# RuanJohn/Mava

Measured on AMD Instinct MI355X. Metric: env-steps/sec (whole node), ff_mappo RWARE tiny-4ag, higher is better.
Workload: dtype f32 via 2 x f16 split operands on the MFMA (3 products, f32 accumulate); 1 GPU; ff_mappo RWARE tiny-4ag-shaped synthetic obs, 4096 envs/GPU (update_batch_size=1 x num_envs=4096), rollout_length=128, ppo_epochs=4, num_minibatches=2, agents=4, obs=70/264, actions=5, one step = one PPO update = 524288 env-steps per GPU; parallelism=dp1

## Files before the change

### include/mava_hip.h

```cpp
#ifndef MAVA_HIP_H
#define MAVA_HIP_H

#include <stddef.h>
#include <stdint.h>

#ifdef __cplusplus
extern "C" {
#endif

typedef struct ihipStream_t* mava_stream_t;

const char* mava_last_error(void);
int mava_abi_version(void);

typedef struct mava_ctx mava_ctx;
enum {
  MAVA_CTX_MATMUL_MODE = 0,
  MAVA_CTX_CRITIC_AGGREGATION = 1,
  MAVA_CTX_GAE_VARIANT = 2,
  MAVA_CTX_POLICY_VARIANT = 3,
  MAVA_CTX_H2_LAUNCHES = 4,
  MAVA_CTX_TRAIN_VARIANT = 5,
  MAVA_CTX_W8_LAUNCHES = 6,
  MAVA_CTX_W1_SPLIT_FRESH = 7,
  MAVA_CTX_EXACT_TILES = 8,
  MAVA_CTX_X16_LAUNCHES = 9,
  MAVA_CTX_X16_W8_LAUNCHES = 10
};
int mava_ctx_create(mava_ctx** out);
int mava_ctx_destroy(mava_ctx* ctx);
int mava_ctx_set(mava_ctx* ctx, int key, long value);
int mava_ctx_get(const mava_ctx* ctx, int key, long* value);

int mava_gae_f32(const mava_ctx* ctx, const float* reward, const float* value, const uint8_t* done,
                 const float* last_val, const uint8_t* last_done, int T, int N, float gamma,
                 float lambda, float* adv, float* tgt, mava_stream_t s);

int mava_permutation_i32(long n, uint64_t seed, uint64_t counter, int32_t* out, mava_stream_t s);
int mava_permutation_batched_i32(long n, uint64_t seed, uint64_t counter, int n_perm, int32_t* out, long out_stride,
                                 mava_stream_t s);

int mava_clip_adam(float* p, const float* g, float* m, float* v, int32_t* count,
                   const int* seg_off, const float* seg_lr, int n_seg, float grad_scale,
                   float max_norm, int decay, int steps_per_update, int num_updates, float b1,
                   float b2, float eps, const float* loss_sums, float vf_coef, float ent_coef,
                   float* metrics_out, mava_stream_t s);

size_t mava_ppo_finish_workspace_bytes(int Pa, int Pc);
int mava_ppo_finish_f32(mava_ctx* ctx, const float* slab_a, long stride_a, const float* slab_c, long stride_c, int n_slab,
                        int Pa, int Pc, float* g, float* p, float* m, float* v, int32_t* count, float lr_a, float lr_c,
// ... 400 lines not shown
```

### mava_amd/_lib.py

```python
from __future__ import annotations

import ctypes as C
import os
from typing import Optional

import torch

_HERE = os.path.dirname(os.path.abspath(__file__))
LIB_PATH = os.environ.get("MAVA_LIB_PATH") or os.path.join(_HERE, "libmavahip.so")

_lib: Optional[C.CDLL] = None


class MavaHipError(RuntimeError):
    pass


vp = C.c_void_p
i32 = C.c_int
u32 = C.c_uint32
u64 = C.c_uint64
f32 = C.c_float
lng = C.c_long

# ... 116 lines not shown
    global _lib
    if _lib is None:
        if not os.path.exists(LIB_PATH):
            raise MavaHipError(
                f"{LIB_PATH} is missing: build it with `python -m mava_amd.build` "
                "(hipcc --offload-arch=gfx950). There is no CPU fallback."
            )
        _lib = C.CDLL(LIB_PATH)
        _lib.mava_last_error.restype = C.c_char_p
        _lib.mava_last_error.argtypes = []
        for name, args in _SIGNATURES.items():
            fn = getattr(_lib, name)
            fn.argtypes = args
            fn.restype = _RESTYPES.get(name, C.c_int)
    return _lib


class Ctx:

    MATMUL_MODE, CRITIC_AGGREGATION, GAE_VARIANT, POLICY_VARIANT, H2_LAUNCHES, TRAIN_VARIANT, W8_LAUNCHES, W1_SPLIT_FRESH = 0, 1, 2, 3, 4, 5, 6, 7
    EXACT_TILES = 8
    X16_LAUNCHES = 9
    X16_W8_LAUNCHES = 10

    def __init__(self, matmul_mode: str = "f32", critic_aggregation: bool = True):
        if matmul_mode not in ("f32", "f16x2"):
            raise ValueError(f"matmul_mode must be 'f16x2' or 'f32', got {matmul_mode!r}")
        h = C.c_void_p()
        check(lib().mava_ctx_create(C.byref(h)), "mava_ctx_create")
        self.handle: Optional[int] = h.value
        self.set(self.MATMUL_MODE, 1 if matmul_mode == "f16x2" else 0)
        self.set(self.CRITIC_AGGREGATION, int(bool(critic_aggregation)))

    def set(self, key: int, value: int) -> None:
        check(lib().mava_ctx_set(self.handle, key, int(value)), "mava_ctx_set")

    def get(self, key: int) -> int:
        out = C.c_long()
        check(lib().mava_ctx_get(self.handle, key, C.byref(out)), "mava_ctx_get")
        return int(out.value)

    @property
    def matmul_mode(self) -> str:
        return "f16x2" if self.get(self.MATMUL_MODE) == 1 else "f32"

    @property
# ... 51 lines not shown
```

### mava_amd/csrc/api.cpp

```cpp
#include <stdarg.h>
#include <stdio.h>
#include <string.h>

#include "common.h"
#include "ctx.h"

static thread_local char g_err[512] = "";

void mava_set_error(const char* fmt, ...) {
  va_list ap;
  va_start(ap, fmt);
  vsnprintf(g_err, sizeof(g_err), fmt, ap);
  va_end(ap);
}

extern "C" const char* mava_last_error(void) { return g_err; }

extern "C" int mava_abi_version(void) { return 3; }

enum { CTX_MATMUL_MODE = 0, CTX_CRITIC_AGGREGATION = 1, CTX_GAE_VARIANT = 2, CTX_POLICY_VARIANT = 3, CTX_H2_LAUNCHES = 4, CTX_TRAIN_VARIANT = 5, CTX_W8_LAUNCHES = 6, CTX_W1_SPLIT_FRESH = 7, CTX_EXACT_TILES = 8, CTX_X16_LAUNCHES = 9, CTX_X16_W8_LAUNCHES = 10 };

extern "C" int mava_ctx_create(mava_ctx** out) {
  MAVA_ARG_CHECK(out != nullptr, 0, "mava_ctx_create: null output pointer");
  mava_ctx* c = new mava_ctx();
  c->matmul_mode = 0;
  c->critic_aggregation = 1;
  c->gae_variant = 0;
  c->policy_variant = 0;
  c->h2_launches = 0;
  c->train_variant = 0;
  c->w8_launches = 0;
  c->w1_split[0] = c->w1_split[1] = nullptr;
  for (int i = 0; i < 2; ++i) {
    c->w1_fresh[i] = 0;
    c->w1_key_params[i] = nullptr;
    c->w1_key_din[i] = c->w1_key_steps[i] = 0;
  }
  c->exact_tiles = nullptr;
  *out = c;
  return MAVA_OK;
}

extern "C" int mava_ctx_destroy(mava_ctx* c) {
// ... 12 lines not shown
      MAVA_ARG_CHECK(value == 0 || value == 1, 1, "mava_ctx_set: matmul mode %ld (0 = exact f32, 1 = f16x2)", value);
      c->matmul_mode = (int)value;
      c->w1_fresh[0] = c->w1_fresh[1] = 0;
      return MAVA_OK;
    case CTX_CRITIC_AGGREGATION: c->critic_aggregation = value ? 1 : 0; return MAVA_OK;
    case CTX_GAE_VARIANT: c->gae_variant = (int)value; return MAVA_OK;
    case CTX_POLICY_VARIANT: c->policy_variant = (int)value; return MAVA_OK;
    case CTX_H2_LAUNCHES: c->h2_launches = value; return MAVA_OK;
    case CTX_TRAIN_VARIANT: c->train_variant = (int)value; return MAVA_OK;
    case CTX_W8_LAUNCHES: c->w8_launches = value; return MAVA_OK;
    case CTX_W1_SPLIT_FRESH:
      MAVA_ARG_CHECK(value == 0, 1, "mava_ctx_set: MAVA_CTX_W1_SPLIT_FRESH can only be cleared (0) by the caller");
      c->w1_fresh[0] = c->w1_fresh[1] = 0;
      return MAVA_OK;
    case CTX_EXACT_TILES:
      MAVA_ARG_CHECK(value == 0, 1, "mava_ctx_set: MAVA_CTX_EXACT_TILES can only be reset (0) by the caller");
      if (c->exact_tiles != nullptr) {
        MAVA_HIP_CHECK(hipDeviceSynchronize());
        MAVA_HIP_CHECK(hipMemset(c->exact_tiles, 0, sizeof(unsigned long long)));
      }
      return MAVA_OK;
    case CTX_X16_LAUNCHES:
    case CTX_X16_W8_LAUNCHES:
      MAVA_ARG_CHECK(value == 0, 1, "mava_ctx_set: MAVA_CTX_X16_LAUNCHES / _W8_LAUNCHES can only be reset (0) by the caller");
      if (c->exact_tiles != nullptr) {
        MAVA_HIP_CHECK(hipDeviceSynchronize());
        MAVA_HIP_CHECK(hipMemset(c->exact_tiles + (key == CTX_X16_W8_LAUNCHES ? 2 : 1), 0, sizeof(unsigned long long)));
      }
      return MAVA_OK;
    default: mava_set_error("mava_ctx_set: unknown key %d", key); return MAVA_EARG(2);
  }
}

extern "C" int mava_ctx_get(const mava_ctx* c, int key, long* value) {
  MAVA_ARG_CHECK(c != nullptr && value != nullptr, 0, "mava_ctx_get: null argument");
  switch (key) {
    case CTX_MATMUL_MODE: *value = c->matmul_mode; return MAVA_OK;
    case CTX_CRITIC_AGGREGATION: *value = c->critic_aggregation; return MAVA_OK;
    case CTX_GAE_VARIANT: *value = c->gae_variant; return MAVA_OK;
    case CTX_POLICY_VARIANT: *value = c->policy_variant; return MAVA_OK;
    case CTX_H2_LAUNCHES: *value = c->h2_launches; return MAVA_OK;
    case CTX_TRAIN_VARIANT: *value = c->train_variant; return MAVA_OK;
    case CTX_W8_LAUNCHES: *value = c->w8_launches; return MAVA_OK;
    case CTX_W1_SPLIT_FRESH: *value = c->w1_fresh[1]; return MAVA_OK;
    case CTX_EXACT_TILES:
    case CTX_X16_LAUNCHES:
    case CTX_X16_W8_LAUNCHES: {
      unsigned long long n = 0;
      if (c->exact_tiles != nullptr) {
        MAVA_HIP_CHECK(hipDeviceSynchronize());
        MAVA_HIP_CHECK(hipMemcpy(&n, c->exact_tiles + (key == CTX_X16_W8_LAUNCHES ? 2 : key == CTX_X16_LAUNCHES ? 1 : 0), sizeof(n), hipMemcpyDeviceToHost));
      }
      *value = (long)n;
      return MAVA_OK;
    }
    default: mava_set_error("mava_ctx_get: unknown key %d", key); return MAVA_EARG(2);
  }
}
```

### mava_amd/csrc/ppo_train_h2.hip

```cpp
#include "h2_core.h"
#include "ppo_train_task.h"
#include "ctx.h"

#include <type_traits>

#ifndef MAVA_GW_DEPTH
#define MAVA_GW_DEPTH 0
#endif
#define GW_DEPTH MAVA_GW_DEPTH
#ifndef MAVA_GW_DEPTH_WIDE
#define MAVA_GW_DEPTH_WIDE 0
#endif
#ifndef MAVA_P1_EARLY_HALVES
#define MAVA_P1_EARLY_HALVES 2
#endif
#ifndef MAVA_P1_EARLY_RING
#define MAVA_P1_EARLY_RING 3
#endif

namespace {

using namespace h2;

constexpr int STATS_BLOCKS = 128;
// ... 1055 lines not shown
      if (tk.x16_valid != nullptr) x16 = __builtin_amdgcn_readfirstlane((int)*tk.x16_valid) == 1;
    }
    if (X16_CAPABLE && x16) {
      if constexpr (X16_CAPABLE) {
        if (threadIdx.x < 256) {
          h2_body<NO, S1, ACTOR, WIDE, XV, 1, true>(tk, L, w1p, lds);
        } else {
          h2_body<NO, S1, ACTOR, WIDE, XV, 2, true>(tk, L, w1p, lds);
        }
      }
    } else if (threadIdx.x < 256) {
      h2_body<NO, S1, ACTOR, WIDE, XV, 1>(tk, L, w1p, lds);
    } else {
      h2_body<NO, S1, ACTOR, WIDE, XV, 2>(tk, L, w1p, lds);
    }
  } else {
    h2_body<NO, S1, ACTOR, WIDE, XV, 0>(tk, L, w1p, lds);
  }
}

int ctx_counters(mava_ctx* ctx, hipStream_t s) {
  if (ctx->exact_tiles == nullptr) {
    void* word = nullptr;
    MAVA_HIP_CHECK(hipMalloc(&word, 3 * sizeof(unsigned long long)));
    ctx->exact_tiles = static_cast<unsigned long long*>(word);
    MAVA_HIP_CHECK(hipMemsetAsync(word, 0, 3 * sizeof(unsigned long long), s));
  }
  return MAVA_OK;
}

template <int NO, int S1, bool ACTOR, bool WIDE, int XV>
int launch_h2(mava_ctx* ctx, const TrainTask& tk, int n_slab, hipStream_t s) {
  const H2Layout L = make_h2_layout<NO, S1, WIDE>(ACTOR);
  MAVA_ARG_CHECK(L.end <= 163840, 8, "ppo_train_h2: %d bytes of LDS exceed the 160 KiB of a CU", L.end);
  static bool attr_set = false;
  if (!attr_set) {
    MAVA_HIP_CHECK(hipFuncSetAttribute((const void*)ppo_train_h2_kernel<NO, S1, ACTOR, WIDE, XV>,
                                       hipFuncAttributeMaxDynamicSharedMemorySize, L.end));
    attr_set = true;
  }
  const uint4* w1p = nullptr;
  if (WIDE) {
    void*& slot = ctx->w1_split[ACTOR ? 0 : 1];
    if (slot == nullptr) MAVA_HIP_CHECK(hipMalloc(&slot, W1_SPLIT_BYTES));
    uint4* const buf = static_cast<uint4*>(slot);
    const int kind = ACTOR ? 0 : 1;
    int& fresh = ctx->w1_fresh[kind];
    const bool keyed = ctx->w1_key_params[kind] == tk.params && ctx->w1_key_din[kind] == tk.din && ctx->w1_key_steps[kind] == S1;
    if (!(fresh && keyed)) {
// ... 46 lines not shown
    default: return 1;
  }
}

}

static int h2_dispatch(mava_ctx* ctx, const TrainTask& tk, int n_slab, bool actor, hipStream_t s) {
  if (actor) {
    if (tk.action_f != nullptr) return 1;
    if (tk.no <= 8) return dispatch_s1<8, true>(ctx, tk, n_slab, s);
#ifndef MAVA_FAST_BUILD
    if (tk.no <= 16) return dispatch_s1<16, true>(ctx, tk, n_slab, s);
    return dispatch_s1<32, true>(ctx, tk, n_slab, s);
#else
    return 1;
#endif
  }
  return dispatch_s1<1, false>(ctx, tk, n_slab, s);
}

int mava_train_h2_launch(mava_ctx* ctx, const TrainTask& tk_in, int n_slab, bool actor, hipStream_t s) {
  TrainTask tk = tk_in;
  tk.force_xlo = (ctx->train_variant & 2) != 0;
  if ((ctx->train_variant & 1) == 0) {
    if (tk.x16 != nullptr && tk.x16_valid != nullptr) {
      const int rcc = ctx_counters(ctx, s);
      if (rcc != MAVA_OK) return rcc;
      tk.x16_launches = ctx->exact_tiles + 2;
    }
    const int rc8 = mava_train_w8_launch(tk, n_slab, actor, s);
    if (rc8 <= 0) {
      if (rc8 == 0) { ++ctx->h2_launches; ++ctx->w8_launches; }
      return rc8;
    }
  }
  const int rc = h2_dispatch(ctx, tk, n_slab, actor, s);
  if (rc == 0) ++ctx->h2_launches;
  return rc;
}
```

### mava_amd/csrc/ppo_train_task.h

```cpp
#pragma once
#include <stdint.h>

#include "common.h"

struct TrainTask {
  const float* params;
  const float* x;
  int din, no, xshare, xv;
  int A;
  int agg;
  const int32_t* idx;
  long idx_base;
  int Rb;
  const uint8_t* mask;
  const int32_t* action;
  const float* action_f;
  uint32_t seed_lo, seed_hi, ent_step, row_offset;
  float min_scale;
  const float* old_logp;
  const float* adv;
  const double* stats;
  const float* old_value;
  const float* targets;
  float clip_eps, ent_coef, vf_coef;
  float* slab;
  long slab_stride;
  unsigned long long* stamps;
  int force_xlo;
  unsigned long long* exact_tiles;
  const _Float16* x16;
  const uint32_t* x16_valid;
  unsigned long long* x16_launches;
  int x16_ld;
};

struct mava_ctx;
int mava_train_w8_launch(const TrainTask& tk, int n_slab, bool actor, hipStream_t s);
int mava_train_h2_launch(mava_ctx* ctx, const TrainTask& tk, int n_slab, bool actor, hipStream_t s);

extern int g_train_last_instance;
constexpr int train_instance_id(int family, bool actor, bool cont, bool wide, int no, int k, int xv) {
  return family * 1000000 + ((actor ? 1 : 0) + (cont ? 2 : 0) + (wide ? 4 : 0)) * 100000 + no * 1000 + k * 10 + xv;
}
```

### mava_amd/csrc/ppo_train_w8.hip

```cpp
#include "h2_core.h"
#include "ppo_train_task.h"
#include "ctx.h"

namespace {

using namespace h2;
typedef float f32x4 __attribute__((ext_vector_type(4)));

constexpr int STATS_BLOCKS = 128;
#ifndef MAVA_W8_GWD
#define MAVA_W8_GWD 1
#endif
constexpr int GWD = MAVA_W8_GWD;

#ifdef MAVA_STAMPS
#define WSTAMP_DECL unsigned long long ws_prev = __builtin_readcyclecounter(), ws_acc[16] = {0, 0, 0, 0, 0, 0, 0, 0, 0, 0, 0, 0, 0, 0, 0, 0};
#define WSTAMP(i)                                                   \
  do {                                                              \
    __builtin_amdgcn_sched_barrier(0);                              \
    const unsigned long long ws_now = __builtin_readcyclecounter(); \
    ws_acc[i] += ws_now - ws_prev;                                  \
    ws_prev = ws_now;                                               \
    __builtin_amdgcn_sched_barrier(0);                              \
  } while (0)
#else
#define WSTAMP_DECL
#define WSTAMP(i)
#endif

struct Frag4 {
  half4 hi, lo;
};
__device__ __forceinline__ f32x4 mfma3w(const Frag& a, const Frag& b, f32x4 c) {
  c = __builtin_amdgcn_mfma_f32_16x16x32_f16(a.lo, b.hi, c, 0, 0, 0);
  c = __builtin_amdgcn_mfma_f32_16x16x32_f16(a.hi, b.lo, c, 0, 0, 0);
  return __builtin_amdgcn_mfma_f32_16x16x32_f16(a.hi, b.hi, c, 0, 0, 0);
// ... 13 lines not shown
}
__device__ __forceinline__ Frag4 split4(const f32x4& v) {
  Frag4 f;
#pragma unroll
  for (int r = 0; r < 4; ++r) {
    _Float16 a, b;
    split1(v[r], a, b);
    f.hi[r] = a;
    f.lo[r] = b;
  }
  return f;
}

constexpr int WROW = 256;
constexpr int WPLANE32 = 32 * WROW;
constexpr int WIMG = 2 * WPLANE32;
constexpr int W2PLANE = 128 * WROW;
constexpr int DYROW = 48;
constexpr int DYPLANE = 32 * DYROW;
__host__ __device__ inline int w8_sw(int row) { return ((row & 3) << 1) | (((row >> 3) & 1) * 9); }
__host__ __device__ inline int w8_off(int row, int chunk) { return WROW * row + 16 * (chunk ^ w8_sw(row)); }

struct W8Layout {
  int h1, dz2, dz1, w2, xs, dy, small, end;
};
inline W8Layout make_w8_layout() {
  W8Layout L;
  L.h1 = 0;
  L.dz2 = L.h1 + WIMG;
  L.dz1 = L.dz2 + WIMG;
  L.w2 = L.dz1 + WIMG;
  L.xs = L.w2 + 2 * W2PLANE;
  L.dy = L.xs + 2 * WIMG;
  L.small = L.dy + 2 * DYPLANE;
  L.end = L.small + (32 + 16 + 16) * 4;
  return L;
}

template <int NO, int S1, int XV, int W2R, bool ACTOR, int ROLE, bool X16 = false>
__device__ __forceinline__ void w8_body(const TrainTask& tk, const W8Layout& L, u8* lds) {
  constexpr bool DO_LOSS = ROLE != 2, DO_STAGE = ROLE != 1;
  static_assert(!X16 || (DO_STAGE && XV == 2), "the f16 record is read by a staging role of an XV = 2 instance");
  constexpr float WS = ACTOR ? 1.0f : W_SCALE_CRITIC, WU = 1.0f / WS;
  constexpr int KT1 = 2 * S1;
  u8* const H1I = lds + L.h1;
  u8* const DZ2I = lds + L.dz2;
  u8* const DZ1I = lds + L.dz1;
  u8* const W2I = lds + L.w2;
  u8* const DYI = lds + L.dy;
  float* const YP = reinterpret_cast<float*>(lds + L.dz2);
  constexpr int YSTR = (NO == 8) ? 9 : NO;
  float* const B3s = reinterpret_cast<float*>(lds + L.small);
  float* const misc = B3s + 32;
  unsigned* const xflag = reinterpret_cast<unsigned*>(misc + 2);

  const int tid = threadIdx.x;
  const int l = tid & 63, v = tid >> 6, i = l & 15, kg = l >> 4;
  const int din = tk.din, no = tk.no;
  const long R = (long)tk.Rb * tk.A;
  const float invR = 1.0f / (float)R;
  const float* const P = tk.params;
  const int oW2 = mlp_off_w2(din), oW3 = mlp_off_w3(din);

  for (int o = tid * 16; o < L.end; o += 512 * 16) *reinterpret_cast<uint4*>(lds + o) = make_uint4(0, 0, 0, 0);
  __syncthreads();
  if (tid < no) B3s[tid] = P[mlp_off_b3(din, no) + tid];
  if (tid < 64) {
    const int b = tid >> 5, row = tid & 31;
    *reinterpret_cast<_Float16*>(lds + L.xs + b * WIMG + w8_off(row, din >> 3) + 2 * (din & 7)) = (_Float16)1.0f;
  }
  {
    const int n = tid & 127, k0 = 32 * (tid >> 7);
    float carry = 0.0f;
#pragma unroll 8
    for (int k = k0; k < k0 + 32; ++k) {
      _Float16 x0, x1;
      split1_carry(P[oW2 + k * MLP_H + n] * WS, carry, x0, x1);
      const int o = w8_off(k, n >> 3) + 2 * (n & 7);
      *reinterpret_cast<_Float16*>(W2I + o) = x0;
      *reinterpret_cast<_Float16*>(W2I + W2PLANE + o) = x1;
    }
  }
  if (ACTOR && tid == 0) {
    double s1 = 0.0, s2 = 0.0;
    for (int b = 0; b < STATS_BLOCKS; ++b) { s1 += tk.stats[2 * b]; s2 += tk.stats[2 * b + 1]; }
    const double mean = s1 / (double)R;
    double var = s2 / (double)R - mean * mean;
    if (var < 0.0) var = 0.0;
    misc[0] = (float)mean;
    misc[1] = 1.0f / ((float)sqrt(var) + 1e-8f);
  }
  Frag W1f[S1], W2f[W2R > 0 ? W2R : 1];
// ... 86 lines not shown
      if (XV == 2) {
        const float2 t = reinterpret_cast<const float2*>(xrow)[cc];
        xr[2 * k] = t.x; xr[2 * k + 1] = t.y;
      } else {
        xr[k] = xrow[cc];
      }
    }
  };
  u8* const xs_dummy = reinterpret_cast<u8*>(misc + 8);
  const int xsw = 16 * w8_sw(srow);
  typedef unsigned u32x4 __attribute__((ext_vector_type(4)));
  typedef const __attribute__((address_space(1))) u32x4* x16_gptr;
  constexpr int NPC16 = (4 * S1 + TPR - 1) / TPR;
  const int rp16 = 8 * ((din + 8) >> 3);
  const int nv16 = (tk.x16_ld < rp16 ? tk.x16_ld : rp16) >> 3;
  auto stage_issue16 = [&](uint32_t fr, u32x4 (&xq)[NPC16]) {
    const x16_gptr xrow = (x16_gptr)(tk.x16 + (long)fr * tk.x16_ld);
#pragma unroll
    for (int k = 0; k < NPC16; ++k) {
      const int c = l16 + TPR * k;
      xq[k] = xrow[(c < nv16) ? c : 0];
    }
  };
  auto stage_commit16 = [&](int buf, const u32x4 (&xq)[NPC16]) {
    u8* base = lds + L.xs + buf * WIMG + WROW * srow;
#pragma unroll
    for (int k = 0; k < NPC16; ++k) {
      const int c = l16 + TPR * k;
      *reinterpret_cast<u32x4*>((c < nv16) ? (base + ((16 * c) ^ xsw)) : xs_dummy) = xq[k];
    }
  };
  auto stage_commit = [&](int buf, const float (&xr)[NR]) {
    u8* base = lds + L.xs + buf * WIMG + WROW * srow;
    uint32_t lo_any = 0;
#pragma unroll
    for (int k = 0; k < NPC; ++k) {
      const int c = l16 + TPR * k;
      const bool ok = c < nv;
      const int col = XV * c;
      u8* qa = ok ? (base + ((16 * (col >> 3)) ^ xsw) + 2 * (col & 7)) : xs_dummy;
      u8* qb = ok ? (qa + WPLANE32) : xs_dummy;
      if (XV == 2) {
        typedef _Float16 half2v __attribute__((ext_vector_type(2)));
        half2v a, b;
#pragma unroll
        for (int e = 0; e < 2; ++e) { _Float16 x0, x1; split1(xr[2 * k + e], x0, x1); a[e] = x0; b[e] = x1; }
        *reinterpret_cast<half2v*>(qa) = a;
        *reinterpret_cast<half2v*>(qb) = b;
// ... 12 lines not shown
    if constexpr (ACTOR) {
      act = tk.action[fr];
      f0 = tk.old_logp[fr];
      f1 = tk.adv[fr];
      const uint8_t* mk = (tk.mask != nullptr && lo < no) ? (tk.mask + (long)fr * no + lo) : nullptr;
      m = 1u;
      if (mk != nullptr) m = *mk;
    } else {
      act = 0;
      f0 = tk.old_value[fr];
      f1 = tk.targets[fr];
      m = 0u;
    }
  };

  const long ntiles = (R + 31) / 32;
  long it = blockIdx.x;
  float xr[X16 ? 1 : NR];
  u32x4 xq[X16 ? NPC16 : 1];
  auto issue = [&](uint32_t fr) __attribute__((always_inline)) {
    if constexpr (X16) stage_issue16(fr, xq); else stage_issue(fr, xr);
  };
  auto commit = [&](int b) __attribute__((always_inline)) {
    if constexpr (X16) stage_commit16(b, xq); else stage_commit(b, xr);
  };
  int r_act = 0, n_act = 0;
  float r_f0 = 0.0f, r_f1 = 0.0f, n_f0 = 0.0f, n_f1 = 0.0f;
  uint32_t r_m = 1u, n_m = 1u;
  Cursor cs = cursor_at(DO_STAGE ? srow : 0), cl = cursor_at(DO_LOSS ? lrow : 0);
  int32_t ps_next = 0, pl_next = 0;
  uint32_t as_next = 0, al_next = 0;
  if (it < ntiles) {
    if constexpr (DO_STAGE) {
      cursor_gather(cs, ps_next, as_next);
      issue(stage_row(ps_next, as_next));
    }
    if constexpr (DO_LOSS) {
      cursor_gather(cl, pl_next, al_next);
      load_row((uint32_t)pl_next * Au + al_next, r_act, r_f0, r_f1, r_m);
    }
    if constexpr (DO_STAGE) {
      commit(0);
      cursor_advance(cs);
    }
    if constexpr (DO_LOSS) cursor_advance(cl);
    if (it + gridDim.x < ntiles) {
      if constexpr (DO_STAGE) { cursor_gather(cs, ps_next, as_next); cursor_advance(cs); }
// ... 9 lines not shown
  const int wrA = WROW * i + 16 * ((2 * v + (kg >> 1)) ^ swi) + 8 * (kg & 1);
  const int tq = i >> 2, tp = i & 3;
  const int trow = 8 * kg + tq;
  const int trb = WROW * trow + 8 * (tp & 1);
  const int thx = 16 * ((tp >> 1) ^ w8_sw(trow));
  int trA[8];
#pragma unroll
  for (int t = 0; t < 8; ++t) {
    trA[t] = trb + ((32 * t) ^ thx);
    asm volatile("" : "+v"(trA[t]));
  }
  auto tr_addr = [&](int t) -> int { return trA[t]; };
  const int trOwn = tr_addr(v);
  auto read_tr = [&](const u8* img, int plane, int a0) -> Frag {
    Frag f;
    f.hi = read_tr8(img + a0, WROW);
    f.lo = read_tr8(img + plane + a0, WROW);
    return f;
  };
  auto read_row = [&](const u8* img, int plane, int a0) -> Frag { return read_row_frag(img, plane, a0); };
  const int dyRd = DYROW * i + 8 * kg;
  const int dyTr = DYROW * trow + 8 * tp;
  int buf = 0;

  WSTAMP_DECL
  for (; it < ntiles; it += gridDim.x, buf ^= 1) {
    WSTAMP(14);
    const long itn = it + gridDim.x;
    const bool have_next = itn < ntiles;
    const u8* const XSI = lds + L.xs + buf * WIMG;
    uint32_t xrow_next = DO_STAGE ? stage_row(ps_next, as_next) : 0u, lrow_next = DO_LOSS ? ((uint32_t)pl_next * Au + al_next) : 0u;
    if constexpr (DO_STAGE) asm volatile("" : "+v"(xrow_next));
    if constexpr (DO_LOSS) asm volatile("" : "+v"(lrow_next));

    f32x4 acc[2] = {f32x4{0, 0, 0, 0}, f32x4{0, 0, 0, 0}};
    const bool x_lo = __builtin_amdgcn_readfirstlane((int)xflag[buf]) != 0 || tk.force_xlo != 0;
    if (x_lo) {
      Frag xb[2];
#pragma unroll
      for (int nt = 0; nt < 2; ++nt) xb[nt] = read_row(XSI + 4096 * nt, WPLANE32, rdA[0]);
#pragma unroll
      for (int s = 0; s < S1; ++s) {
        Frag b[2] = {xb[0], xb[1]};
        if (s + 1 < S1) {
#pragma unroll
          for (int nt = 0; nt < 2; ++nt) xb[nt] = read_row(XSI + 4096 * nt, WPLANE32, rdA[(s + 1) & 3]);
        }
#pragma unroll
        for (int nt = 0; nt < 2; ++nt) acc[nt] = mfma3w(W1f[s], b[nt], acc[nt]);
        __builtin_amdgcn_sched_barrier(0);
      }
    } else {
      half8 xb[2];
#pragma unroll
      for (int nt = 0; nt < 2; ++nt) xb[nt] = *reinterpret_cast<const half8*>(XSI + 4096 * nt + rdA[0]);
#pragma unroll
      for (int s = 0; s < S1; ++s) {
        const half8 b[2] = {xb[0], xb[1]};
        if (s + 1 < S1) {
// ... 46 lines not shown
      for (int s = 0; s < 4; ++s) {
        Frag b[2] = {hb[0], hb[1]};
        const Frag a = (s < W2R) ? W2f[s < W2R ? s : 0] : wn;
        if (s + 1 < 4) {
#pragma unroll
          for (int nt = 0; nt < 2; ++nt) hb[nt] = read_row(H1I + 4096 * nt, WPLANE32, rdA[s + 1]);
          if (s + 1 >= W2R) wn = read_tr(W2I + 32 * (s + 1) * WROW, W2PLANE, trOwn);
        }
#pragma unroll
        for (int nt = 0; nt < 2; ++nt) h2[nt] = mfma3w(a, b[nt], h2[nt]);
        __builtin_amdgcn_sched_barrier(0);
      }
    }
    WSTAMP(4);
    uint32_t relu2 = 0;
#pragma unroll
    for (int nt = 0; nt < 2; ++nt) {
#pragma unroll
      for (int r = 0; r < 4; ++r) {
        h2[nt][r] = fmaxf(ACTOR ? h2[nt][r] : h2[nt][r] * WU, 0.0f);
        relu2 |= (h2[nt][r] > 0.0f) ? (1u << (4 * nt + r)) : 0u;
      }
      const Frag4 f = split4(h2[nt]);
      *reinterpret_cast<half4*>(DZ1I + 4096 * nt + wrA) = f.hi;
      *reinterpret_cast<half4*>(DZ1I + 4096 * nt + WPLANE32 + wrA) = f.lo;
      const f32x4 y = mfma3k16(W3h, f, f32x4{0, 0, 0, 0});
#pragma unroll
      for (int r = 0; r < 4; ++r) {
        if (4 * kg + r < NO) YP[(v * 32 + 16 * nt + i) * YSTR + 4 * kg + r] = y[r] * W3_UNSCALE;
      }
    }
    WSTAMP(5);
    __syncthreads();
    WSTAMP(6);

    if constexpr (DO_LOSS) {
      const float lo_c = 1.0f - tk.clip_eps, hi_c = 1.0f + tk.clip_eps;
      const bool rvalid = (it * 32 + lrow) < R;
      const float* yp = YP + lrow * YSTR + lo;
      float y = B3s[lo];
#pragma unroll
      for (int u = 0; u < 8; ++u) y += yp[u * 32 * YSTR];
      float dyo = 0.0f, pg_row = 0.0f, ent_row = 0.0f;
      if constexpr (ACTOR) {
        const bool legal = (lo < no) && (r_m != 0u);
        const float z = legal ? y : -FLT_MAX;
        auto fmax_op = [](float a, float b) { return fmaxf(a, b); };
        auto add_op = [](float a, float b) { return a + b; };
        const float mx = group_allreduce<NO>(z, fmax_op);
        const float se = group_allreduce<NO>(expf(z - mx), add_op);
        const float logp = (mx == -FLT_MAX) ? ((lo < no) ? -logf((float)no) : -FLT_MAX) : z - (mx + logf(se));
        const float pr = expf(logp);
        const float ent = group_allreduce<NO>((pr > 0.0f) ? -(pr * logp) : 0.0f, add_op);
        const int act = r_act;
        const float lp = group_allreduce<NO>((lo == act) ? logp : 0.0f, add_op);
        const float gae = (r_f1 - adv_mean) * adv_rstd;
        const float ratio = expf(lp - r_f0);
        const float rc = fminf(fmaxf(ratio, lo_c), hi_c);
// ... 14 lines not shown
        const float ov = r_f0, tg = r_f1;
        const float diff = y - ov;
        const float vclip = ov + fminf(fmaxf(diff, -tk.clip_eps), tk.clip_eps);
        const float e1 = y - tg, e2 = vclip - tg;
        const float l1 = e1 * e1, l2 = e2 * e2;
        const bool inside = (diff >= -tk.clip_eps) && (diff <= tk.clip_eps);
        const float g1 = (l1 > l2) ? 1.0f : ((l1 == l2) ? 0.5f : 0.0f);
        const float g2 = inside ? (1.0f - g1) : 0.0f;
        dyo = (rvalid && lo == 0) ? (tk.vf_coef * (g1 * e1 + g2 * e2)) : 0.0f;
        pg_row = 0.5f * fmaxf(l1, l2);
      }
      _Float16 da, db;
      split1(dyo, da, db);
      *reinterpret_cast<_Float16*>(DYI + lrow * DYROW + 2 * lo) = da;
      *reinterpret_cast<_Float16*>(DYI + DYPLANE + lrow * DYROW + 2 * lo) = db;
      ab3 += dyo;
      if (rvalid && lo == 0) {
        loss_a += pg_row * invR;
        loss_b += ent_row * invR;
      }
      r_act = n_act; r_f0 = n_f0; r_f1 = n_f1; r_m = n_m;
    }
    if constexpr (DO_STAGE) {
      if (have_next) commit(buf ^ 1);
    }
    WSTAMP(7);
    __syncthreads();
    WSTAMP(8);

    {
      Frag a, b;
      a.hi = read_tr8(DYI + dyTr, DYROW);
      a.lo = read_tr8(DYI + DYPLANE + dyTr, DYROW);
      b = read_tr(DZ1I, WPLANE32, trOwn);
      gW3 = mfma3w(a, b, gW3);
    }
    f32x4 dz[2];
#pragma unroll
    for (int nt = 0; nt < 2; ++nt) {
      Frag4 b;
      b.hi = *reinterpret_cast<const half4*>(DYI + 16 * nt * DYROW + dyRd);
      b.lo = *reinterpret_cast<const half4*>(DYI + DYPLANE + 16 * nt * DYROW + dyRd);
      dz[nt] = mfma3k16(W3d, b, f32x4{0, 0, 0, 0});
#pragma unroll
      for (int r = 0; r < 4; ++r) {
        dz[nt][r] = ((relu2 >> (4 * nt + r)) & 1u) ? dz[nt][r] * W3_UNSCALE : 0.0f;
        ab2[r] += dz[nt][r];
      }
      const Frag4 f = split4(dz[nt]);
      *reinterpret_cast<half4*>(DZ2I + 4096 * nt + wrA) = f.hi;
      *reinterpret_cast<half4*>(DZ2I + 4096 * nt + WPLANE32 + wrA) = f.lo;
    }
    WSTAMP(9);
    {
      const Frag b = read_tr(DZ2I, WPLANE32, trOwn);
      Frag an[GWD];
#pragma unroll
// ... 20 lines not shown
#pragma unroll
      for (int s = 0; s < 4; ++s) {
        const Frag a = an;
        Frag b[2] = {bn[0], bn[1]};
        if (s + 1 < 4) {
          an = read_row(W2I + 4096 * v, W2PLANE, rdA[s + 1]);
#pragma unroll
          for (int nt = 0; nt < 2; ++nt) bn[nt] = read_row(DZ2I + 4096 * nt, WPLANE32, rdA[s + 1]);
        }
#pragma unroll
        for (int nt = 0; nt < 2; ++nt) acc[nt] = mfma3w(a, b[nt], acc[nt]);
        __builtin_amdgcn_sched_barrier(0);
      }
#pragma unroll
      for (int nt = 0; nt < 2; ++nt) {
#pragma unroll
        for (int r = 0; r < 4; ++r) acc[nt][r] = ((relu1 >> (4 * nt + r)) & 1u) ? (ACTOR ? acc[nt][r] : acc[nt][r] * WU) : 0.0f;
        const Frag4 f = split4(acc[nt]);
        *reinterpret_cast<half4*>(DZ1I + 4096 * nt + wrA) = f.hi;
        *reinterpret_cast<half4*>(DZ1I + 4096 * nt + WPLANE32 + wrA) = f.lo;
      }
    }
    WSTAMP(12);
    {
      const Frag b = read_tr(DZ1I, WPLANE32, trOwn);
      constexpr int D1 = GWD < KT1 ? GWD : KT1;
      if (x_lo) {
        Frag an[D1];
#pragma unroll
        for (int t = 0; t < D1; ++t) an[t] = read_tr(XSI, WPLANE32, tr_addr(t));
#pragma unroll
        for (int t = 0; t < KT1; ++t) {
          const Frag a = an[t % D1];
          if (t + D1 < KT1) an[t % D1] = read_tr(XSI, WPLANE32, tr_addr(t + D1));
          gW1[t] = mfma3w(a, b, gW1[t]);
          __builtin_amdgcn_sched_barrier(0);
        }
      } else {
        half8 an[D1];
#pragma unroll
        for (int t = 0; t < D1; ++t) an[t] = read_tr8(XSI + tr_addr(t), WROW);
#pragma unroll
        for (int t = 0; t < KT1; ++t) {
          const half8 a = an[t % D1];
          if (t + D1 < KT1) an[t % D1] = read_tr8(XSI + tr_addr(t + D1), WROW);
          gW1[t] = mfma2w_alo0(a, b, gW1[t]);
          __builtin_amdgcn_sched_barrier(0);
        }
      }
    }
    WSTAMP(13);
  }
#ifdef MAVA_STAMPS
  if (tk.stamps != nullptr && blockIdx.x == 0 && l == 0) {
    for (int k = 0; k < 16; ++k) tk.stamps[v * 16 + k] = ws_acc[k];
  }
#endif

  __syncthreads();
  if constexpr (X16) {
    if (st == 0 && blockIdx.x == 0 && tk.x16_launches != nullptr) atomicAdd(tk.x16_launches, 1ull);
  }
  float* slab = tk.slab + (long)blockIdx.x * tk.slab_stride;
  const int oB2 = mlp_off_b2(din), oB3 = mlp_off_b3(din, no);
  const int Pn = mlp_param_count(din, no);
#pragma unroll
  for (int t = 0; t < KT1; ++t)
#pragma unroll
    for (int r = 0; r < 4; ++r) {
      const int k = 16 * t + 4 * kg + r;
      if (k <= din) slab[k * MLP_H + 16 * v + i] = gW1[t][r] * invR;
    }
#pragma unroll
  for (int t = 0; t < 8; ++t)
#pragma unroll
    for (int r = 0; r < 4; ++r) slab[oW2 + (16 * t + 4 * kg + r) * MLP_H + 16 * v + i] = gW2[t][r] * invR;
#pragma unroll
  for (int r = 0; r < 4; ++r) {
    float x = ab2[r];
#pragma unroll
    for (int m = 1; m < 16; m <<= 1) x += __shfl_xor(x, m, 64);
    if (i == 0) slab[oB2 + 16 * v + 4 * kg + r] = x * invR;
    const int o = 4 * kg + r;
    if (o < no) slab[oW3 + (16 * v + i) * no + o] = gW3[r] * invR;
// ... 19 lines not shown
    slab[oB3 + tid] = x * invR;
  }
  if (tid == 0) {
    float a = 0.0f, b = 0.0f;
#pragma unroll
    for (int u = 0; u < LW; ++u) { a += red[8 * NO + 2 * u]; b += red[8 * NO + 2 * u + 1]; }
    slab[Pn] = a;
    slab[Pn + 1] = b;
  }
}

constexpr int w8_w2r(int no, int s1, int xv) {
#ifdef MAVA_W8_W2R
  return MAVA_W8_W2R;
#else
  return (no == 8) ? ((s1 <= 2) ? 2 : ((s1 == 3 && xv == 2) ? 2 : 0)) : ((s1 <= 2) ? 2 : 0);
#endif
}
template <int NO, int S1, int XV, int W2R, bool ACTOR>
__global__ __launch_bounds__(512, 2) void ppo_train_w8_kernel(TrainTask tk, W8Layout L) {
  extern __shared__ __attribute__((aligned(16))) u8 lds[];
  constexpr bool X16_CAPABLE = XV == 2;
  if constexpr (NO == 8) {
    if (threadIdx.x < 256) {
      w8_body<NO, S1, XV, W2R, ACTOR, 1>(tk, L, lds);
    } else {
      bool x16 = false;
      if constexpr (X16_CAPABLE) {
        if (tk.x16_valid != nullptr) x16 = __builtin_amdgcn_readfirstlane((int)*tk.x16_valid) == 1;
      }
      if (X16_CAPABLE && x16) {
        if constexpr (X16_CAPABLE) w8_body<NO, S1, XV, W2R, ACTOR, 2, true>(tk, L, lds);
      } else {
        w8_body<NO, S1, XV, W2R, ACTOR, 2>(tk, L, lds);
      }
    }
  } else {
    bool x16 = false;
    if constexpr (X16_CAPABLE) {
      if (tk.x16_valid != nullptr) x16 = __builtin_amdgcn_readfirstlane((int)*tk.x16_valid) == 1;
    }
    if (X16_CAPABLE && x16) {
      if constexpr (X16_CAPABLE) w8_body<NO, S1, XV, W2R, ACTOR, 0, true>(tk, L, lds);
    } else {
      w8_body<NO, S1, XV, W2R, ACTOR, 0>(tk, L, lds);
    }
  }
}

template <int NO, int S1, int XV, bool ACTOR>
int launch_w8(const TrainTask& tk, int n_slab, hipStream_t s) {
  const W8Layout L = make_w8_layout();
  static bool attr_set = false;
  if (!attr_set) {
    MAVA_HIP_CHECK(hipFuncSetAttribute((const void*)ppo_train_w8_kernel<NO, S1, XV, w8_w2r(NO, S1, XV), ACTOR>, hipFuncAttributeMaxDynamicSharedMemorySize,
                                       L.end));
    attr_set = true;
  }
  TrainTask tkl = tk;
  const int ld16 = tk.x16_ld != 0 ? tk.x16_ld : tk.din;
  const bool x16_ok = XV == 2 && tk.x16 != nullptr && tk.x16_valid != nullptr && ld16 % 8 == 0 && ld16 >= tk.din &&
                      (uintptr_t)tk.x16 % 16 == 0 && tk.force_xlo == 0 && tk.xshare == 1 && tk.agg <= 1;
  tkl.x16_ld = ld16;
  if (!x16_ok) { tkl.x16 = nullptr; tkl.x16_valid = nullptr; tkl.x16_launches = nullptr; }
  g_train_last_instance = train_instance_id(3, ACTOR, false, false, NO, S1, XV);
  hipLaunchKernelGGL((ppo_train_w8_kernel<NO, S1, XV, w8_w2r(NO, S1, XV), ACTOR>), dim3(n_slab), dim3(512), L.end, s, tkl, L);
  MAVA_LAUNCH_CHECK();
  return MAVA_OK;
}

template <int NO, int S1, bool ACTOR>
int dispatch_w8_xv(const TrainTask& tk, int n_slab, hipStream_t s) {
  if (tk.din % 2 == 0 && ((uintptr_t)tk.x) % 8 == 0) return launch_w8<NO, S1, 2, ACTOR>(tk, n_slab, s);
  if constexpr (S1 == 4) return 1;
  else return launch_w8<NO, S1, 1, ACTOR>(tk, n_slab, s);
}

template <int NO, bool ACTOR>
int dispatch_w8(const TrainTask& tk, int n_slab, hipStream_t s) {
  const int s1 = (tk.din + 1 + 31) / 32;
  switch (s1) {
#ifndef MAVA_FAST_BUILD
    case 1: return dispatch_w8_xv<NO, 1, ACTOR>(tk, n_slab, s);
    case 2: return dispatch_w8_xv<NO, 2, ACTOR>(tk, n_slab, s);
    case 4: return dispatch_w8_xv<NO, 4, ACTOR>(tk, n_slab, s);
#endif
    case 3: return dispatch_w8_xv<NO, 3, ACTOR>(tk, n_slab, s);
// ... 19 lines not shown
```

Baseline: 84.87 million env-steps/s.

## Defer dW1 accumulation by one tile in role-split w8 training kernel

Adds a deferred-dW1 mode to the role-split (NO==8, f16-record) w8 training kernel. The input staging buffer becomes a three-slot ring and h2 gets its own LDS planes, so the dW1 MFMA product for the previous tile can run inside the loss/staging phases of the current tile instead of serializing at the tile tail. This is meant to balance work between the loss and staging wave groups and hide dW1 behind other phases, at the cost of extra LDS (a third x plane plus h2 planes), which could reduce occupancy. The mode is on by default and can be disabled via a train_variant bit, with a launch counter added for verification.

```diff
diff --git a/include/mava_hip.h b/include/mava_hip.h
--- a/include/mava_hip.h
+++ b/include/mava_hip.h
@@ -25,7 +25,8 @@
   MAVA_CTX_W1_SPLIT_FRESH = 7,
   MAVA_CTX_EXACT_TILES = 8,
   MAVA_CTX_X16_LAUNCHES = 9,
-  MAVA_CTX_X16_W8_LAUNCHES = 10
+  MAVA_CTX_X16_W8_LAUNCHES = 10,
+  MAVA_CTX_W8_DEFER_LAUNCHES = 11
 };
 int mava_ctx_create(mava_ctx** out);
 int mava_ctx_destroy(mava_ctx* ctx);
diff --git a/mava_amd/_lib.py b/mava_amd/_lib.py
--- a/mava_amd/_lib.py
+++ b/mava_amd/_lib.py
@@ -162,6 +162,7 @@
     EXACT_TILES = 8
     X16_LAUNCHES = 9
     X16_W8_LAUNCHES = 10
+    W8_DEFER_LAUNCHES = 11
 
     def __init__(self, matmul_mode: str = "f32", critic_aggregation: bool = True):
         if matmul_mode not in ("f32", "f16x2"):
diff --git a/mava_amd/csrc/api.cpp b/mava_amd/csrc/api.cpp
--- a/mava_amd/csrc/api.cpp
+++ b/mava_amd/csrc/api.cpp
@@ -18,7 +18,7 @@
 
 extern "C" int mava_abi_version(void) { return 3; }
 
-enum { CTX_MATMUL_MODE = 0, CTX_CRITIC_AGGREGATION = 1, CTX_GAE_VARIANT = 2, CTX_POLICY_VARIANT = 3, CTX_H2_LAUNCHES = 4, CTX_TRAIN_VARIANT = 5, CTX_W8_LAUNCHES = 6, CTX_W1_SPLIT_FRESH = 7, CTX_EXACT_TILES = 8, CTX_X16_LAUNCHES = 9, CTX_X16_W8_LAUNCHES = 10 };
+enum { CTX_MATMUL_MODE = 0, CTX_CRITIC_AGGREGATION = 1, CTX_GAE_VARIANT = 2, CTX_POLICY_VARIANT = 3, CTX_H2_LAUNCHES = 4, CTX_TRAIN_VARIANT = 5, CTX_W8_LAUNCHES = 6, CTX_W1_SPLIT_FRESH = 7, CTX_EXACT_TILES = 8, CTX_X16_LAUNCHES = 9, CTX_X16_W8_LAUNCHES = 10, CTX_W8_DEFER_LAUNCHES = 11 };
 
 extern "C" int mava_ctx_create(mava_ctx** out) {
   MAVA_ARG_CHECK(out != nullptr, 0, "mava_ctx_create: null output pointer");
@@ -77,10 +77,11 @@
       return MAVA_OK;
     case CTX_X16_LAUNCHES:
     case CTX_X16_W8_LAUNCHES:
-      MAVA_ARG_CHECK(value == 0, 1, "mava_ctx_set: MAVA_CTX_X16_LAUNCHES / _W8_LAUNCHES can only be reset (0) by the caller");
+    case CTX_W8_DEFER_LAUNCHES:
+      MAVA_ARG_CHECK(value == 0, 1, "mava_ctx_set: MAVA_CTX_X16_LAUNCHES / _W8_LAUNCHES / MAVA_CTX_W8_DEFER_LAUNCHES can only be reset (0) by the caller");
       if (c->exact_tiles != nullptr) {
         MAVA_HIP_CHECK(hipDeviceSynchronize());
-        MAVA_HIP_CHECK(hipMemset(c->exact_tiles + (key == CTX_X16_W8_LAUNCHES ? 2 : 1), 0, sizeof(unsigned long long)));
+        MAVA_HIP_CHECK(hipMemset(c->exact_tiles + (key == CTX_W8_DEFER_LAUNCHES ? 3 : key == CTX_X16_W8_LAUNCHES ? 2 : 1), 0, sizeof(unsigned long long)));
       }
       return MAVA_OK;
     default: mava_set_error("mava_ctx_set: unknown key %d", key); return MAVA_EARG(2);
@@ -100,11 +101,12 @@
     case CTX_W1_SPLIT_FRESH: *value = c->w1_fresh[1]; return MAVA_OK;
     case CTX_EXACT_TILES:
     case CTX_X16_LAUNCHES:
-    case CTX_X16_W8_LAUNCHES: {
+    case CTX_X16_W8_LAUNCHES:
+    case CTX_W8_DEFER_LAUNCHES: {
       unsigned long long n = 0;
       if (c->exact_tiles != nullptr) {
         MAVA_HIP_CHECK(hipDeviceSynchronize());
-        MAVA_HIP_CHECK(hipMemcpy(&n, c->exact_tiles + (key == CTX_X16_W8_LAUNCHES ? 2 : key == CTX_X16_LAUNCHES ? 1 : 0), sizeof(n), hipMemcpyDeviceToHost));
+        MAVA_HIP_CHECK(hipMemcpy(&n, c->exact_tiles + (key == CTX_W8_DEFER_LAUNCHES ? 3 : key == CTX_X16_W8_LAUNCHES ? 2 : key == CTX_X16_LAUNCHES ? 1 : 0), sizeof(n), hipMemcpyDeviceToHost));
       }
       *value = (long)n;
       return MAVA_OK;
diff --git a/mava_amd/csrc/ppo_train_h2.hip b/mava_amd/csrc/ppo_train_h2.hip
--- a/mava_amd/csrc/ppo_train_h2.hip
+++ b/mava_amd/csrc/ppo_train_h2.hip
@@ -1101,9 +1101,9 @@
 int ctx_counters(mava_ctx* ctx, hipStream_t s) {
   if (ctx->exact_tiles == nullptr) {
     void* word = nullptr;
-    MAVA_HIP_CHECK(hipMalloc(&word, 3 * sizeof(unsigned long long)));
+    MAVA_HIP_CHECK(hipMalloc(&word, 4 * sizeof(unsigned long long)));
     ctx->exact_tiles = static_cast<unsigned long long*>(word);
-    MAVA_HIP_CHECK(hipMemsetAsync(word, 0, 3 * sizeof(unsigned long long), s));
+    MAVA_HIP_CHECK(hipMemsetAsync(word, 0, 4 * sizeof(unsigned long long), s));
   }
   return MAVA_OK;
 }
@@ -1196,11 +1196,13 @@
 int mava_train_h2_launch(mava_ctx* ctx, const TrainTask& tk_in, int n_slab, bool actor, hipStream_t s) {
   TrainTask tk = tk_in;
   tk.force_xlo = (ctx->train_variant & 2) != 0;
+  tk.no_defer = (ctx->train_variant & 4) != 0;
   if ((ctx->train_variant & 1) == 0) {
     if (tk.x16 != nullptr && tk.x16_valid != nullptr) {
       const int rcc = ctx_counters(ctx, s);
       if (rcc != MAVA_OK) return rcc;
       tk.x16_launches = ctx->exact_tiles + 2;
+      tk.defer_launches = ctx->exact_tiles + 3;
     }
     const int rc8 = mava_train_w8_launch(tk, n_slab, actor, s);
     if (rc8 <= 0) {
diff --git a/mava_amd/csrc/ppo_train_task.h b/mava_amd/csrc/ppo_train_task.h
--- a/mava_amd/csrc/ppo_train_task.h
+++ b/mava_amd/csrc/ppo_train_task.h
@@ -32,6 +32,8 @@
   const uint32_t* x16_valid;
   unsigned long long* x16_launches;
   int x16_ld;
+  int no_defer;
+  unsigned long long* defer_launches;
 };
 
 struct mava_ctx;
diff --git a/mava_amd/csrc/ppo_train_w8.hip b/mava_amd/csrc/ppo_train_w8.hip
--- a/mava_amd/csrc/ppo_train_w8.hip
+++ b/mava_amd/csrc/ppo_train_w8.hip
@@ -12,6 +12,11 @@
 #define MAVA_W8_GWD 1
 #endif
 constexpr int GWD = MAVA_W8_GWD;
+#ifndef MAVA_W8_DEFER
+#define MAVA_W8_DEFER 1
+#endif
+constexpr int W8_DEFER = MAVA_W8_DEFER;
+static_assert(W8_DEFER >= 0 && W8_DEFER <= 2, "MAVA_W8_DEFER is 0, 1 or 2");
 
 #ifdef MAVA_STAMPS
 #define WSTAMP_DECL unsigned long long ws_prev = __builtin_readcyclecounter(), ws_acc[16] = {0, 0, 0, 0, 0, 0, 0, 0, 0, 0, 0, 0, 0, 0, 0, 0};
@@ -71,7 +76,7 @@
 __host__ __device__ inline int w8_off(int row, int chunk) { return WROW * row + 16 * (chunk ^ w8_sw(row)); }
 
 struct W8Layout {
-  int h1, dz2, dz1, w2, xs, dy, small, end;
+  int h1, dz2, dz1, w2, xs, dy, small, h2hi, h2lo, end;
 };
 inline W8Layout make_w8_layout() {
   W8Layout L;
@@ -82,14 +87,18 @@
   L.xs = L.w2 + 2 * W2PLANE;
   L.dy = L.xs + 2 * WIMG;
   L.small = L.dy + 2 * DYPLANE;
-  L.end = L.small + (32 + 16 + 16) * 4;
+  L.h2hi = L.xs + 3 * WPLANE32;
+  L.h2lo = (L.small + (32 + 16 + 16) * 4 + 15) & ~15;
+  L.end = L.h2lo + WPLANE32;
   return L;
 }
 
-template <int NO, int S1, int XV, int W2R, bool ACTOR, int ROLE, bool X16 = false>
+template <int NO, int S1, int XV, int W2R, bool ACTOR, int ROLE, bool X16 = false, int DF = 0>
 __device__ __forceinline__ void w8_body(const TrainTask& tk, const W8Layout& L, u8* lds) {
   constexpr bool DO_LOSS = ROLE != 2, DO_STAGE = ROLE != 1;
   static_assert(!X16 || (DO_STAGE && XV == 2), "the f16 record is read by a staging role of an XV = 2 instance");
+  static_assert(DF == 0 || (NO == 8 && XV == 2 && (ROLE == 1 || (ROLE == 2 && X16 && DF == 2))),
+                "the deferred-dW1 form belongs to the role-split instances on the f16 record; its staging role always defers");
   constexpr float WS = ACTOR ? 1.0f : W_SCALE_CRITIC, WU = 1.0f / WS;
   constexpr int KT1 = 2 * S1;
   u8* const H1I = lds + L.h1;
@@ -97,6 +106,8 @@
   u8* const DZ1I = lds + L.dz1;
   u8* const W2I = lds + L.w2;
   u8* const DYI = lds + L.dy;
+  u8* const H2HI = lds + (DF != 0 ? L.h2hi : L.dz1);
+  u8* const H2LO = lds + (DF != 0 ? L.h2lo : L.dz1 + WPLANE32);
   float* const YP = reinterpret_cast<float*>(lds + L.dz2);
   constexpr int YSTR = (NO == 8) ? 9 : NO;
   float* const B3s = reinterpret_cast<float*>(lds + L.small);
@@ -114,9 +125,9 @@
   for (int o = tid * 16; o < L.end; o += 512 * 16) *reinterpret_cast<uint4*>(lds + o) = make_uint4(0, 0, 0, 0);
   __syncthreads();
   if (tid < no) B3s[tid] = P[mlp_off_b3(din, no) + tid];
-  if (tid < 64) {
+  if (tid < (DF != 0 ? 96 : 64)) {
     const int b = tid >> 5, row = tid & 31;
-    *reinterpret_cast<_Float16*>(lds + L.xs + b * WIMG + w8_off(row, din >> 3) + 2 * (din & 7)) = (_Float16)1.0f;
+    *reinterpret_cast<_Float16*>(lds + L.xs + b * (DF != 0 ? WPLANE32 : WIMG) + w8_off(row, din >> 3) + 2 * (din & 7)) = (_Float16)1.0f;
   }
   {
     const int n = tid & 127, k0 = 32 * (tid >> 7);
@@ -249,8 +260,8 @@
       xq[k] = xrow[(c < nv16) ? c : 0];
     }
   };
-  auto stage_commit16 = [&](int buf, const u32x4 (&xq)[NPC16]) {
-    u8* base = lds + L.xs + buf * WIMG + WROW * srow;
+  auto stage_commit16 = [&](int xo, const u32x4 (&xq)[NPC16]) {
+    u8* base = lds + L.xs + xo + WROW * srow;
 #pragma unroll
     for (int k = 0; k < NPC16; ++k) {
       const int c = l16 + TPR * k;
@@ -309,7 +320,7 @@
     if constexpr (X16) stage_issue16(fr, xq); else stage_issue(fr, xr);
   };
   auto commit = [&](int b) __attribute__((always_inline)) {
-    if constexpr (X16) stage_commit16(b, xq); else stage_commit(b, xr);
+    if constexpr (X16) stage_commit16(DF != 0 ? b : b * WIMG, xq); else stage_commit(b, xr);
   };
   int r_act = 0, n_act = 0;
   float r_f0 = 0.0f, r_f1 = 0.0f, n_f0 = 0.0f, n_f1 = 0.0f;
@@ -365,19 +376,31 @@
   const int dyRd = DYROW * i + 8 * kg;
   const int dyTr = DYROW * trow + 8 * tp;
   int buf = 0;
+  int xo_cur = 0, xo_nxt = WPLANE32, xo_prv = 2 * WPLANE32;
+  auto dw1_exact = [&](const u8* xsi) __attribute__((always_inline)) {
+    const Frag b = read_tr(DZ1I, WPLANE32, trOwn);
+    half8 a[KT1];
+#pragma unroll
+    for (int t = 0; t < KT1; ++t) a[t] = read_tr8(xsi + tr_addr(t), WROW);
+#pragma unroll
+    for (int t = 0; t < KT1; ++t) gW1[t] = __builtin_amdgcn_mfma_f32_16x16x32_f16(a[t], b.lo, gW1[t], 0, 0, 0);
+#pragma unroll
+    for (int t = 0; t < KT1; ++t) gW1[t] = __builtin_amdgcn_mfma_f32_16x16x32_f16(a[t], b.hi, gW1[t], 0, 0, 0);
+  };
 
   WSTAMP_DECL
   for (; it < ntiles; it += gridDim.x, buf ^= 1) {
     WSTAMP(14);
     const long itn = it + gridDim.x;
     const bool have_next = itn < ntiles;
-    const u8* const XSI = lds + L.xs + buf * WIMG;
+    const bool first_tile = it == (long)blockIdx.x;
+    const u8* const XSI = lds + L.xs + (DF != 0 ? xo_cur : buf * WIMG);
     uint32_t xrow_next = DO_STAGE ? stage_row(ps_next, as_next) : 0u, lrow_next = DO_LOSS ? ((uint32_t)pl_next * Au + al_next) : 0u;
     if constexpr (DO_STAGE) asm volatile("" : "+v"(xrow_next));
     if constexpr (DO_LOSS) asm volatile("" : "+v"(lrow_next));
 
     f32x4 acc[2] = {f32x4{0, 0, 0, 0}, f32x4{0, 0, 0, 0}};
-    const bool x_lo = __builtin_amdgcn_readfirstlane((int)xflag[buf]) != 0 || tk.force_xlo != 0;
+    const bool x_lo = DF == 0 && (__builtin_amdgcn_readfirstlane((int)xflag[buf]) != 0 || tk.force_xlo != 0);
     if (x_lo) {
       Frag xb[2];
 #pragma unroll
@@ -470,8 +493,8 @@
         relu2 |= (h2[nt][r] > 0.0f) ? (1u << (4 * nt + r)) : 0u;
       }
       const Frag4 f = split4(h2[nt]);
-      *reinterpret_cast<half4*>(DZ1I + 4096 * nt + wrA) = f.hi;
-      *reinterpret_cast<half4*>(DZ1I + 4096 * nt + WPLANE32 + wrA) = f.lo;
+      *reinterpret_cast<half4*>(H2HI + 4096 * nt + wrA) = f.hi;
+      *reinterpret_cast<half4*>(H2LO + 4096 * nt + wrA) = f.lo;
       const f32x4 y = mfma3k16(W3h, f, f32x4{0, 0, 0, 0});
 #pragma unroll
       for (int r = 0; r < 4; ++r) {
@@ -482,6 +505,10 @@
     __syncthreads();
     WSTAMP(6);
 
+    if constexpr (DO_LOSS && DF == 2) {
+      if (!first_tile) dw1_exact(lds + L.xs + xo_prv);
+      WSTAMP(15);
+    }
     if constexpr (DO_LOSS) {
       const float lo_c = 1.0f - tk.clip_eps, hi_c = 1.0f + tk.clip_eps;
       const bool rvalid = (it * 32 + lrow) < R;
@@ -542,9 +569,13 @@
       r_act = n_act; r_f0 = n_f0; r_f1 = n_f1; r_m = n_m;
     }
     if constexpr (DO_STAGE) {
-      if (have_next) commit(buf ^ 1);
+      if (have_next) commit(DF != 0 ? xo_nxt : (buf ^ 1));
     }
     WSTAMP(7);
+    if constexpr (DO_STAGE && DF == 2) {
+      if (!first_tile) dw1_exact(lds + L.xs + xo_prv);
+      WSTAMP(15);
+    }
     __syncthreads();
     WSTAMP(8);
 
@@ -552,7 +583,8 @@
       Frag a, b;
       a.hi = read_tr8(DYI + dyTr, DYROW);
       a.lo = read_tr8(DYI + DYPLANE + dyTr, DYROW);
-      b = read_tr(DZ1I, WPLANE32, trOwn);
+      b.hi = read_tr8(H2HI + trOwn, WROW);
+      b.lo = read_tr8(H2LO + trOwn, WROW);
       gW3 = mfma3w(a, b, gW3);
     }
     f32x4 dz[2];
@@ -619,7 +651,10 @@
       }
     }
     WSTAMP(12);
-    {
+    if constexpr (DF == 2) {
+    } else if constexpr (DF == 1) {
+      dw1_exact(XSI);
+    } else {
       const Frag b = read_tr(DZ1I, WPLANE32, trOwn);
       constexpr int D1 = GWD < KT1 ? GWD : KT1;
       if (x_lo) {
@@ -647,6 +682,14 @@
       }
     }
     WSTAMP(13);
+    if constexpr (DF != 0) {
+      const int t = xo_prv;
+      xo_prv = xo_cur; xo_cur = xo_nxt; xo_nxt = t;
+    }
+  }
+  if constexpr (DF == 2) {
+    if ((long)blockIdx.x < ntiles) dw1_exact(lds + L.xs + xo_prv);
+    WSTAMP(15);
   }
 #ifdef MAVA_STAMPS
   if (tk.stamps != nullptr && blockIdx.x == 0 && l == 0) {
@@ -657,6 +700,9 @@
   __syncthreads();
   if constexpr (X16) {
     if (st == 0 && blockIdx.x == 0 && tk.x16_launches != nullptr) atomicAdd(tk.x16_launches, 1ull);
+    if constexpr (DF == 2) {
+      if (st == 0 && blockIdx.x == 0 && tk.defer_launches != nullptr) atomicAdd(tk.defer_launches, 1ull);
+    }
   }
   float* slab = tk.slab + (long)blockIdx.x * tk.slab_stride;
   const int oB2 = mlp_off_b2(din), oB3 = mlp_off_b3(din, no);
@@ -722,7 +768,17 @@
   extern __shared__ __attribute__((aligned(16))) u8 lds[];
   constexpr bool X16_CAPABLE = XV == 2;
   if constexpr (NO == 8) {
-    if (threadIdx.x < 256) {
+    constexpr bool DEFER_CAPABLE = X16_CAPABLE && W8_DEFER != 0;
+    bool defer = false;
+    if constexpr (DEFER_CAPABLE) {
+      if (tk.x16_valid != nullptr && tk.no_defer == 0) defer = __builtin_amdgcn_readfirstlane((int)*tk.x16_valid) == 1;
+    }
+    if (DEFER_CAPABLE && defer) {
+      if constexpr (DEFER_CAPABLE) {
+        if (threadIdx.x < 256) w8_body<NO, S1, XV, W2R, ACTOR, 1, false, W8_DEFER>(tk, L, lds);
+        else w8_body<NO, S1, XV, W2R, ACTOR, 2, true, 2>(tk, L, lds);
+      }
+    } else if (threadIdx.x < 256) {
       w8_body<NO, S1, XV, W2R, ACTOR, 1>(tk, L, lds);
     } else {
       bool x16 = false;
@@ -751,6 +807,7 @@
 template <int NO, int S1, int XV, bool ACTOR>
 int launch_w8(const TrainTask& tk, int n_slab, hipStream_t s) {
   const W8Layout L = make_w8_layout();
+  MAVA_ARG_CHECK(L.end <= 163840, 8, "ppo_train_w8: %d bytes of LDS exceed the 160 KiB of a CU", L.end);
   static bool attr_set = false;
   if (!attr_set) {
     MAVA_HIP_CHECK(hipFuncSetAttribute((const void*)ppo_train_w8_kernel<NO, S1, XV, w8_w2r(NO, S1, XV), ACTOR>, hipFuncAttributeMaxDynamicSharedMemorySize,
@@ -762,7 +819,7 @@
   const bool x16_ok = XV == 2 && tk.x16 != nullptr && tk.x16_valid != nullptr && ld16 % 8 == 0 && ld16 >= tk.din &&
                       (uintptr_t)tk.x16 % 16 == 0 && tk.force_xlo == 0 && tk.xshare == 1 && tk.agg <= 1;
   tkl.x16_ld = ld16;
-  if (!x16_ok) { tkl.x16 = nullptr; tkl.x16_valid = nullptr; tkl.x16_launches = nullptr; }
+  if (!x16_ok) { tkl.x16 = nullptr; tkl.x16_valid = nullptr; tkl.x16_launches = nullptr; tkl.defer_launches = nullptr; }
   g_train_last_instance = train_instance_id(3, ACTOR, false, false, NO, S1, XV);
   hipLaunchKernelGGL((ppo_train_w8_kernel<NO, S1, XV, w8_w2r(NO, S1, XV), ACTOR>), dim3(n_slab), dim3(512), L.end, s, tkl, L);
   MAVA_LAUNCH_CHECK();
```

Measured after the change: 87.64 million env-steps/s, median of 6. 1.03x the previous value.
